# RQLuo/CDLNet-video

Hardware: AMD Instinct MI355X
Metric: Mpix/s denoised (fwd+bwd) at K=30,M=64,P=7 (higher is better)
Workload: dtype f32 (split-bf16 x3 MFMA, fp32 accumulate, fp32 storage)

## Files before the change

cdlnet-video_amd/csrc/cdl_fused2d.hip:

```cpp
#include <atomic>
#include <cstdlib>
#include <type_traits>
#include <mutex>
#include <utility>
#include <vector>

#include "cdl_common.h"
#include "cdl_fused_sweep.h"


namespace {

#include "cdl_wave_dev.h"

typedef __attribute__((ext_vector_type(4))) __bf16 bf16x4;

constexpr int WX = 2;
constexpr int RB = 8;
constexpr int TW = 32 * WX;
constexpr int HALO = 3;
constexpr int RTW = TW + 2 * HALO;
constexpr int RTC = RTW + 2;
constexpr int LDS_W = 32 * 64 * 16;
constexpr int LDS_TAU = 64 * 4;

constexpr int GW_TH = 16;
constexpr int GW_RTH = GW_TH + 2 * HALO;
constexpr int TROWS = GW_RTH + 1;
constexpr int TPITCH = 72;
constexpr int TCOPY = TROWS * TPITCH;
constexpr int WG_THIN_BYTES = 2 * 2 * 4 * TCOPY * 2;
constexpr int IMG_ELEMS = 32 * 32;

template <int WY_>
struct Shape {
    static_assert(WY_ == 2 || WY_ == 4, "64 x 16 or 64 x 32 tiles");
    static constexpr int WY = WY_;
    static constexpr int NW = WX * WY;
    static constexpr int NT = 64 * NW;
    static constexpr int TH = RB * WY;
    static constexpr int RTH = TH + 2 * HALO;
    static constexpr int PITCH = WY == 2 ? 28 : 44;
    static constexpr int COPY = RTC * PITCH;
    static constexpr int LDS_RT = 2 * 4 * COPY * 2;
    static constexpr int SLAB = RTH * RTW;
    static constexpr int LDS_RSUM = 4 * SLAB * 4;
    static constexpr int LDS_TACC = NW * 64 * 4;
    static constexpr int LDS_STAGE = LDS_RT + LDS_RSUM + LDS_W + LDS_TAU + LDS_TACC;
    static constexpr int LDS_DA_THIN = 2 * 4 * TCOPY * 2;
    static constexpr int LDS_DA = LDS_DA_THIN + NW * 2 * 2 * IMG_ELEMS * 2;
    static constexpr int NSTG = (RTH * RTW + NT - 1) / NT;
    static constexpr bool WREG = WY == 2;
};

struct FusedParams {
    const float *r;
    const float *zin;
    unsigned *map;
    float *zout;
    const float *tau;
    float *dtau;
    const uint4 *frags;
    float *patches;
    float sgn;
    int do_synth;
    CDL_DBG_FIELD(int dbg;)
    int N, H, W, tilesX, tilesY;
    int rev;
    const float *r2;
    float *da_partial;
};

__device__ __forceinline__ float embed7(const float *w, int P, int i, int j)
{
    const int off = (7 - P) / 2;
    const int ii = i - off, jj = j - off;
    if (i > 6 || j > 6 || ii < 0 || jj < 0 || ii >= P || jj >= P) return 0.0f;
    return w[ii * P + jj];
}

__device__ __forceinline__ void prep_one(const float *__restrict__ wA, const float *__restrict__ wB,
                                         uint4 *__restrict__ out, int MT, int P, int t)
{
    const int FA = MT * 4, FB = 4 * MT;
    if (t >= (FA + FB) * 64) return;
    const int lane = t & 63, f = t >> 6;
    const int row = lane & 31, h = lane >> 5;
    const int PP = P * P;
    float v[8];
    if (f < FA) {
        const int R = f / 4, ks = f % 4;
        const int ch = 32 * R + row;
#pragma unroll
        for (int jj = 0; jj < 8; ++jj) v[jj] = embed7(wA + (size_t)ch * PP, P, jj, 2 * ks + h);
    } else {
        const int g = f - FA;
        const int Rp = g / (2 * MT), ksB = g % (2 * MT);
        const int R = ksB >> 1, s = ksB & 1;
        const int tap = 32 * Rp + row;
#pragma unroll
        for (int jj = 0; jj < 8; ++jj) {
            const int ch = 32 * R + 16 * s + 8 * (jj >> 2) + 4 * h + (jj & 3);
            v[jj] = embed7(wB + (size_t)ch * PP, P, tap >> 3, tap & 7);
        }
    }
    bf16x8 hi, lo;
#pragma unroll
    for (int jj = 0; jj < 8; ++jj) {
        __bf16 hh = (__bf16)v[jj];
        hi[jj] = hh;
        lo[jj] = (__bf16)(v[jj] - (float)hh);
    }
    uint4 *hi_dst, *lo_dst;
    if (f < FA) { hi_dst = out + (size_t)f * 64; lo_dst = out + (size_t)(FA + f) * 64; }
    else { hi_dst = out + (size_t)(2 * FA + (f - FA)) * 64; lo_dst = out + (size_t)(2 * FA + FB + (f - FA)) * 64; }
    hi_dst[lane] = __builtin_bit_cast(uint4, hi);
    lo_dst[lane] = __builtin_bit_cast(uint4, lo);
}

__global__ void k_prep(const float *__restrict__ wA, const float *__restrict__ wB,
                       uint4 *__restrict__ out, int MT, int P)
{
    prep_one(wA, wB, out, MT, P, blockIdx.x * blockDim.x + threadIdx.x);
}

constexpr int PREP_BATCH = 32;
struct PrepBatch {
    const float *wA[PREP_BATCH];
    const float *wB[PREP_BATCH];
};
__global__ void k_prep_batch(PrepBatch b, uint4 *__restrict__ out, int frag_uint4, int MT, int P)
{
    prep_one(b.wA[blockIdx.y], b.wB[blockIdx.y], out + (size_t)blockIdx.y * frag_uint4, MT, P,
             blockIdx.x * blockDim.x + threadIdx.x);
}

#ifndef CDL_FAT_LD_AUX
#define CDL_FAT_LD_AUX 0
#endif
#ifndef CDL_FAT_ST_AUX
#define CDL_FAT_ST_AUX 0
#endif
__device__ __forceinline__ __amdgpu_buffer_rsrc_t fat_rsrc(const float *base, size_t img_floats)
{
    return __builtin_amdgcn_make_buffer_rsrc(const_cast<float *>(base), 0, (int)(img_floats * 4), 0x00020000);
}
__device__ __forceinline__ float buf_ld(__amdgpu_buffer_rsrc_t r, int voff, int soff)
{
    return __builtin_bit_cast(float, __builtin_amdgcn_raw_buffer_load_b32(r, voff, soff, CDL_FAT_LD_AUX));
}
__device__ __forceinline__ void buf_st(float v, __amdgpu_buffer_rsrc_t r, int voff, int soff)
{
    __builtin_amdgcn_raw_buffer_store_b32(__builtin_bit_cast(unsigned, v), r, voff, soff, CDL_FAT_ST_AUX);
// ... 17 lines not shown
    return __builtin_amdgcn_make_buffer_rsrc(b, 0, __builtin_amdgcn_readfirstlane((int)bytes), 0x00020000);
}

__device__ __forceinline__ float bf16_round(float v) { return (float)(__bf16)v; }

template <int MT>
__device__ __forceinline__ void blk16_load_raw(u32x2 (&z)[MT][4], __amdgpu_buffer_rsrc_t rs, int voff)
{
#pragma unroll
    for (int R = 0; R < MT; ++R)
#pragma unroll
        for (int q = 0; q < 4; ++q)
            z[R][q] = __builtin_bit_cast(u32x2, __builtin_amdgcn_raw_buffer_load_b64(rs, voff, (8 * R + 2 * q) * 32 * 8, CDL_FAT_LD_AUX));
}
__device__ __forceinline__ float blk16_decode(const u32x2 &u, int e)
{
    const unsigned w = (e & 2) ? u.y : u.x;
    return __builtin_bit_cast(float, (e & 1) ? (w & 0xffff0000u) : (w << 16));
}

template <int LAY, int MT>
__device__ __forceinline__ void blk_load(float (&z)[MT][16], __amdgpu_buffer_rsrc_t rs, int voff)
{
    constexpr int EB = LAY == LAY_BLK ? 16 : 8;
#pragma unroll
    for (int R = 0; R < MT; ++R)
#pragma unroll
        for (int q = 0; q < 4; ++q) {
            const int soff = (8 * R + 2 * q) * 32 * EB;
            if constexpr (LAY == LAY_BLK) {
                typedef __attribute__((ext_vector_type(4))) float f32x4;
                const f32x4 f = __builtin_bit_cast(f32x4, __builtin_amdgcn_raw_buffer_load_b128(rs, voff, soff, CDL_FAT_LD_AUX));
                z[R][4 * q + 0] = f.x; z[R][4 * q + 1] = f.y; z[R][4 * q + 2] = f.z; z[R][4 * q + 3] = f.w;
            } else {
                const u32x2 u = __builtin_bit_cast(u32x2, __builtin_amdgcn_raw_buffer_load_b64(rs, voff, soff, CDL_FAT_LD_AUX));
                z[R][4 * q + 0] = __builtin_bit_cast(float, u.x << 16);
                z[R][4 * q + 1] = __builtin_bit_cast(float, u.x & 0xffff0000u);
                z[R][4 * q + 2] = __builtin_bit_cast(float, u.y << 16);
                z[R][4 * q + 3] = __builtin_bit_cast(float, u.y & 0xffff0000u);
            }
        }
}
template <int LAY>
__device__ __forceinline__ void blk_store4(float a0, float a1, float a2, float a3, __amdgpu_buffer_rsrc_t rs, int voff, int quad_pair)
{
    constexpr int EB = LAY == LAY_BLK ? 16 : 8;
    const int soff = quad_pair * 32 * EB;
    if constexpr (LAY == LAY_BLK) {
        typedef __attribute__((ext_vector_type(4))) float f32x4;
        const f32x4 f = {a0, a1, a2, a3};
        __builtin_amdgcn_raw_buffer_store_b128(__builtin_bit_cast(u32x4, f), rs, voff, soff, CDL_FAT_ST_AUX);
    } else {
        u32x2 u;
        u.x = (__builtin_bit_cast(unsigned, a0) >> 16) | (__builtin_bit_cast(unsigned, a1) & 0xffff0000u);
        u.y = (__builtin_bit_cast(unsigned, a2) >> 16) | (__builtin_bit_cast(unsigned, a3) & 0xffff0000u);
        __builtin_amdgcn_raw_buffer_store_b64(u, rs, voff, soff, CDL_FAT_ST_AUX);
    }
}

template <int N>
__device__ __forceinline__ float lane_transpose_sum(const float (&v)[N], int c)
{
    float r = LaneTransposeSum<N>::run(v, c);
    if (N == 16) r += __shfl_xor(r, 16, 64);
    return r;
}

__device__ __forceinline__ float col2im_row(const float (&rv)[4], int h)
{
    const float r4 = upper_half_to_lower(rv[0]);
    const float r5 = upper_half_to_lower(rv[1]);
    const float r6 = upper_half_to_lower(rv[2]);
    const bool lo = h == 0;
    float s = lo ? r6 : 0.0f;
    s = wave_shr1(s) + (lo ? r5 : 0.0f);
    s = wave_shr1(s) + (lo ? r4 : 0.0f);
    s = wave_shr1(s) + (lo ? rv[3] : 0.0f);
    s = wave_shr1(s) + (lo ? rv[2] : 0.0f);
    s = wave_shr1(s) + (lo ? rv[1] : 0.0f);
    s = wave_shr1(s) + (lo ? rv[0] : 0.0f);
    return s;
}

template <int MT, int PREC, int MODE, int LIN, int LOUT, bool DA = false, int WY = 2>
__global__ __launch_bounds__(Shape<WY>::NT) void k_stage(FusedParams p)
{
    using G = Shape<WY>;
    constexpr int NW = G::NW, NT = G::NT, TH = G::TH, RTH = G::RTH, PITCH = G::PITCH, COPY = G::COPY, SLAB = G::SLAB;
    constexpr int LDS_RT = G::LDS_RT, LDS_RSUM = G::LDS_RSUM, LDS_STAGE = G::LDS_STAGE, LDS_DA_THIN = G::LDS_DA_THIN;
    static_assert(!DA || (MODE == MODE_BWD && TH == GW_TH), "dA_k rides in the reverse stage, on k_wgrad2d's 64 x 16 tiles");
    extern __shared__ __attribute__((aligned(16))) unsigned char smem[];
    __bf16 *rt = reinterpret_cast<__bf16 *>(smem);
    float *rsum_all = reinterpret_cast<float *>(smem + LDS_RT);
    const uint4 *wl = reinterpret_cast<const uint4 *>(smem + LDS_RT + LDS_RSUM);
    float *tau_s = reinterpret_cast<float *>(smem + LDS_RT + LDS_RSUM + LDS_W);
    float *tacc_s = tau_s + 64;
    __bf16 *thin2 = reinterpret_cast<__bf16 *>(smem + LDS_STAGE);
    __bf16 *imgs2 = reinterpret_cast<__bf16 *>(smem + LDS_STAGE + LDS_DA_THIN);

    constexpr int M = 32 * MT;
    constexpr int FA = MT * 4, FB = 4 * MT;
    constexpr int NFRAG = (PREC != 1 ? 2 : 1) * (FA + FB);
    constexpr int NSTG = G::NSTG;
    const int tid = threadIdx.x, lane = tid & 63, wid = tid >> 6;
    const int wxi = wid % WX, wyi = wid / WX;
    const int c = lane & 31, h = lane >> 5;
    const size_t HW = (size_t)p.H * p.W;
    const int numTiles = p.N * p.tilesY * p.tilesX;

    {
        uint4 *z4 = reinterpret_cast<uint4 *>(smem);
        for (int i = tid; i < (LDS_RT + LDS_RSUM) / 16; i += NT) z4[i] = make_uint4(0, 0, 0, 0);
        uint4 *wdst = reinterpret_cast<uint4 *>(smem + LDS_RT + LDS_RSUM);
        if (PREC != 1) {
            for (int i = tid; i < NFRAG * 64; i += NT) wdst[i] = p.frags[i];
        } else {
            for (int i = tid; i < FA * 64; i += NT) wdst[i] = p.frags[i];
            for (int i = tid; i < FB * 64; i += NT) wdst[FA * 64 + i] = p.frags[2 * FA * 64 + i];
        }
    }
    float stg[NSTG];
    auto stage_load = [&](int t) {
        int bid = p.rev ? numTiles - 1 - t : t;
        const int txi = bid % p.tilesX; bid /= p.tilesX;
        const int tyi = bid % p.tilesY;
        const int n = bid / p.tilesY;
        const float *rimg = p.r + (size_t)n * HW;
#pragma unroll
        for (int k = 0; k < NSTG; ++k) {
            const int i = tid + k * NT;
            const int yy = i / RTW, xx = i % RTW;
            const int gy = tyi * TH - HALO + yy, gx = txi * TW - HALO + xx;
            float v = 0.0f;
            if (i < RTH * RTW && t < numTiles && !CDL_DBG(p.dbg, 8) && gy >= 0 && gy < p.H && gx >= 0 && gx < p.W)
                v = rimg[(size_t)gy * p.W + gx];
            stg[k] = v;
        }
    };
    auto stage_store = [&]() {
#pragma unroll
        for (int k = 0; k < NSTG; ++k) {
            const int i = tid + k * NT;
            if (i >= RTH * RTW) continue;
            const int yy = i / RTW, xx = i % RTW;
            const __bf16 hh = (__bf16)stg[k];
            const __bf16 ll = (__bf16)(stg[k] - (float)hh);
#pragma unroll
            for (int q = 0; q < 4; ++q)
                if (yy - q >= 0) {
                    rt[(0 * 4 + q) * COPY + xx * PITCH + (yy - q)] = hh;
                    if (PREC != 1) rt[(1 * 4 + q) * COPY + xx * PITCH + (yy - q)] = ll;
                }
        }
    };
    constexpr int NSTG2 = DA ? (GW_RTH * RTW + NT - 1) / NT : 1;
    float stg2[NSTG2];
    auto stage2_load = [&](int t) {
        int bid = p.rev ? numTiles - 1 - t : t;
        const int txi = bid % p.tilesX; bid /= p.tilesX;
        const int tyi = bid % p.tilesY;
        const int n = bid / p.tilesY;
        const float *timg = p.r2 + (t < numTiles ? (size_t)n * HW : 0);
#pragma unroll
        for (int k = 0; k < NSTG2; ++k) {
            const int i = tid + k * NT;
            const int yy = i / RTW, xx = i % RTW;
            const int gy = tyi * TH - HALO + yy, gx = txi * TW - HALO + xx;
            const bool ok = i < GW_RTH * RTW && t < numTiles && gy >= 0 && gy < p.H && gx >= 0 && gx < p.W;
            const float v = timg[ok ? (size_t)gy * p.W + gx : 0];
            stg2[k] = ok ? v : 0.0f;
        }
    };
    auto stage2_store = [&]() {
#pragma unroll
        for (int k = 0; k < NSTG2; ++k) {
            const int i = tid + k * NT;
            if (i >= GW_RTH * RTW) continue;
            const int yy = i / RTW, xx = i % RTW;
            const __bf16 hh = (__bf16)stg2[k];
            const __bf16 ll = (__bf16)(stg2[k] - (float)hh);
#pragma unroll
            for (int sft = 0; sft < 4; ++sft)
                if (xx - sft >= 0) {
                    thin2[(0 * 4 + sft) * TCOPY + yy * TPITCH + xx - sft] = hh;
                    if (PREC != 1) thin2[(1 * 4 + sft) * TCOPY + yy * TPITCH + xx - sft] = ll;
                }
        }
    };
    f32x16 dacc[DA ? MT : 1][2];
    if constexpr (DA) {
#pragma unroll
        for (int R = 0; R < MT; ++R)
#pragma unroll
            for (int tt = 0; tt < 2; ++tt)
#pragma unroll
                for (int v = 0; v < 16; ++v) dacc[R][tt][v] = 0.0f;
        for (int i = tid; i < LDS_DA_THIN / 16; i += NT) reinterpret_cast<uint4 *>(thin2)[i] = make_uint4(0, 0, 0, 0);
        stage2_load(blockIdx.x);
    }
    stage_load(blockIdx.x);
    __syncthreads();
    stage_store();
    if constexpr (DA) stage2_store();

    constexpr int OFF_AH = 0;
    constexpr int OFF_AL = FA;
    constexpr int OFF_BH = (PREC != 1 ? 2 * FA : FA);
    constexpr int OFF_BL = 2 * FA + FB;
    constexpr bool WREG = G::WREG;
    bf16x8 wreg[WREG ? NFRAG : 1];
    if constexpr (WREG) {
#pragma unroll
        for (int f = 0; f < NFRAG; ++f) wreg[f] = __builtin_bit_cast(bf16x8, wl[f * 64 + lane]);
    }
    auto wfrag = [&](int f) __attribute__((always_inline)) {
        if constexpr (WREG) return wreg[f];
        else return __builtin_bit_cast(bf16x8, wl[f * 64 + lane]);
    };

    const int xl = wxi * 32 + c;
    float *rsum = rsum_all + ((wxi & 1) + 2 * (wyi & 1)) * SLAB;
    const bool has_base = (MODE == MODE_FWD) || (MODE == MODE_BWD && p.zin != nullptr);
    const int hw4 = (int)HW * 4;

#pragma unroll 1
    for (int t = blockIdx.x; t < numTiles; t += gridDim.x) {
    const int tile = p.rev ? numTiles - 1 - t : t;
    int bid = tile;
    const int txi = bid % p.tilesX; bid /= p.tilesX;
    const int tyi = bid % p.tilesY;
    const int n = bid / p.tilesY;
    const int tx0 = txi * TW, ty0 = tyi * TH;
    const int x = tx0 + xl;
    if (MODE != MODE_BWD && tid < M) tau_s[tid] = p.tau[(size_t)n * M + tid];
    __syncthreads();
    if (MODE != MODE_BWD) stage_load(t + gridDim.x);

    float ring[7][4];
#pragma unroll
    for (int i = 0; i < 7; ++i)
#pragma unroll
        for (int j = 0; j < 4; ++j) ring[i][j] = 0.0f;
    float tsum[MT * 16];
#pragma unroll
    for (int i = 0; i < MT * 16; ++i) tsum[i] = 0.0f;
    const bool tau_neg = MODE != MODE_BWD && __ballot(lane < M && !(tau_s[lane] >= 0.0f)) != 0ull;
    float taur[MT * 16];
    if (MODE != MODE_BWD) {
#pragma unroll
        for (int R = 0; R < MT; ++R)
#pragma unroll
            for (int qv = 0; qv < 4; ++qv) {
                const float4 t4 = *reinterpret_cast<const float4 *>(&tau_s[32 * R + 8 * qv + 4 * h]);
                taur[16 * R + 4 * qv + 0] = t4.x; taur[16 * R + 4 * qv + 1] = t4.y;
                taur[16 * R + 4 * qv + 2] = t4.z; taur[16 * R + 4 * qv + 3] = t4.w;
            }
    }

    const bool xok = x < p.W;
    const size_t img_in = lay_image_bytes<LIN>(M, p.H, p.W), img_out = lay_image_bytes<LOUT>(M, p.H, p.W);
    const __amdgpu_buffer_rsrc_t rs_in = uniform_rsrc(
        has_base ? (const char *)p.zin + (size_t)n * img_in : (const char *)p.zout, has_base ? img_in : 0);
    unsigned *const map_n = p.map ? p.map + ((size_t)n * 4 + 2 * h) * HW : nullptr;
    const __amdgpu_buffer_rsrc_t rs_out = uniform_rsrc((const char *)p.zout + (size_t)n * img_out, img_out);
    const int lane_off = (int)((4 * h) * HW + x) * 4;
    const int XB = (p.W + 31) / 32, xb = (tx0 >> 5) + wxi;
    constexpr int EB_IN = LIN == LAY_BLK16 ? 8 : 16, EB_OUT = LOUT == LAY_BLK16 ? 8 : 16;
    const int lane_blk_in = (h * 32 + c) * EB_IN, lane_blk_out = (h * 32 + c) * EB_OUT;

#pragma unroll 1
    for (int b = 0; b < RB; ++b) {
        const int yl = wyi * RB + b;
        const int y = ty0 + yl;
        const bool valid = xok && (y < p.H);
        const int voff = valid ? lane_off + y * p.W * 4 : OOB;
        const int blk = (y * XB + xb) * (M / 4) * 32;
        const int voff_in = LIN == LAY_NCHW ? voff : (valid ? blk * EB_IN + lane_blk_in : OOB);
        const int voff_st = CDL_DBG(p.dbg, 1) ? OOB : (LOUT == LAY_NCHW ? voff : (valid ? blk * EB_OUT + lane_blk_out : OOB));

        float zc[MT][16];
        u32x2 zr[MT][4];
        if (MODE != MODE_FIRST && LIN == LAY_BLK16) {
            blk16_load_raw<MT>(zr, rs_in, voff_in);
        } else if (MODE != MODE_FIRST && CDL_DBG(p.dbg, 16)) {
#pragma unroll
            for (int R = 0; R < MT; ++R)
#pragma unroll
                for (int v = 0; v < 16; ++v) zc[R][v] = 0.25f;
        } else if (MODE != MODE_FIRST && LIN != LAY_NCHW) {
            blk_load<LIN, MT>(zc, rs_in, voff_in);
        } else if (MODE != MODE_FIRST) {
#pragma unroll
            for (int R = 0; R < MT; ++R)
#pragma unroll
                for (int v = 0; v < 16; ++v) {
                    const int soff = (32 * R + 8 * (v >> 2) + (v & 3)) * hw4;
                    zc[R][v] = buf_ld(rs_in, voff, soff);
                }
        }
        unsigned sup = 0, sgb = 0;
        if (MODE == MODE_BWD && valid) {
            sup = map_n[(size_t)y * p.W + x];
            sgb = map_n[HW + (size_t)y * p.W + x];
        }

        const int q = b & 3, e = yl - q;
        bf16x8 rh[4], rl[4];
#pragma unroll
        for (int ks = 0; ks < 4; ++ks) {
            const int col = xl + 2 * ks + h;
            const __bf16 *ph = rt + (0 * 4 + q) * COPY + col * PITCH + e;
            const bf16x4 a0 = *reinterpret_cast<const bf16x4 *>(ph);
            const bf16x4 a1 = *reinterpret_cast<const bf16x4 *>(ph + 4);
            rh[ks] = __builtin_shufflevector(a0, a1, 0, 1, 2, 3, 4, 5, 6, 7);
            if (PREC != 1) {
                const __bf16 *pl = rt + (1 * 4 + q) * COPY + col * PITCH + e;
                const bf16x4 b0 = *reinterpret_cast<const bf16x4 *>(pl);
                const bf16x4 b1 = *reinterpret_cast<const bf16x4 *>(pl + 4);
                rl[ks] = __builtin_shufflevector(b0, b1, 0, 1, 2, 3, 4, 5, 6, 7);
            }
        }

        __builtin_amdgcn_sched_barrier(0);
        f32x16 acc[MT];
#pragma unroll
        for (int R = 0; R < MT; ++R)
#pragma unroll
            for (int v = 0; v < 16; ++v) acc[R][v] = 0.0f;
        if CDL_DBG(p.dbg, 4) {
#pragma unroll
            for (int R = 0; R < MT; ++R) acc[R][0] = (float)rh[0][0] + (float)rl[1][1];
        } else {
            bf16x8 wh[2][MT], wlo[2][MT];
#pragma unroll
            for (int R = 0; R < MT; ++R) {
                wh[0][R] = wfrag(OFF_AH + R * 4);
                if (PREC != 1) wlo[0][R] = wfrag(OFF_AL + R * 4);
            }
#pragma unroll
            for (int ks = 0; ks < 4; ++ks) {
                const int cu = ks & 1, nx = cu ^ 1;
                if (ks + 1 < 4) {
#pragma unroll
                    for (int R = 0; R < MT; ++R) {
                        wh[nx][R] = wfrag(OFF_AH + R * 4 + ks + 1);
                        if (PREC != 1) wlo[nx][R] = wfrag(OFF_AL + R * 4 + ks + 1);
                    }
                }
                if (PREC != 1) {
#pragma unroll
                    for (int R = 0; R < MT; ++R) acc[R] = __builtin_amdgcn_mfma_f32_32x32x16_bf16(wlo[cu][R], rh[ks], acc[R], 0, 0, 0);
#pragma unroll
                    for (int R = 0; R < MT; ++R) acc[R] = __builtin_amdgcn_mfma_f32_32x32x16_bf16(wh[cu][R], rl[ks], acc[R], 0, 0, 0);
                    if (PREC == 2) {
#pragma unroll
                        for (int R = 0; R < MT; ++R) acc[R] = __builtin_amdgcn_mfma_f32_32x32x16_bf16(wlo[cu][R], rl[ks], acc[R], 0, 0, 0);
                    }
                }
#pragma unroll
                for (int R = 0; R < MT; ++R) acc[R] = __builtin_amdgcn_mfma_f32_32x32x16_bf16(wh[cu][R], rh[ks], acc[R], 0, 0, 0);
            }
// ... 128 lines not shown
        __builtin_amdgcn_sched_barrier(0);
        f32x16 D[2];
#pragma unroll
        for (int Rp = 0; Rp < 2; ++Rp)
#pragma unroll
            for (int v = 0; v < 16; ++v) D[Rp][v] = 0.0f;
        {
            bf16x8 bwh[2][2], bwl[2][2];
#pragma unroll
            for (int Rp = 0; Rp < 2; ++Rp) {
                bwh[0][Rp] = wfrag(OFF_BH + Rp * 2 * MT);
                if (PREC != 1) bwl[0][Rp] = wfrag(OFF_BL + Rp * 2 * MT);
            }
#pragma unroll
            for (int q = 0; q < 2 * MT; ++q) {
                const int R = q >> 1, s = q & 1, cu = q & 1, nx = cu ^ 1;
                if (q + 1 < 2 * MT) {
#pragma unroll
                    for (int Rp = 0; Rp < 2; ++Rp) {
                        bwh[nx][Rp] = wfrag(OFF_BH + Rp * 2 * MT + q + 1);
                        if (PREC != 1) bwl[nx][Rp] = wfrag(OFF_BL + Rp * 2 * MT + q + 1);
                    }
                }
                bf16x8 zh, zl;
#pragma unroll
                for (int jj = 0; jj < 8; ++jj) {
                    const float val = acc[R][8 * s + jj];
                    const __bf16 hh = (__bf16)val;
                    zh[jj] = hh;
                    if (PREC != 1 && LOUT != LAY_BLK16) zl[jj] = (__bf16)(val - (float)hh);
                }
                if (PREC != 1) {
#pragma unroll
                    for (int Rp = 0; Rp < 2; ++Rp) D[Rp] = __builtin_amdgcn_mfma_f32_32x32x16_bf16(bwl[cu][Rp], zh, D[Rp], 0, 0, 0);
                    if (LOUT != LAY_BLK16) {
#pragma unroll
                        for (int Rp = 0; Rp < 2; ++Rp) D[Rp] = __builtin_amdgcn_mfma_f32_32x32x16_bf16(bwh[cu][Rp], zl, D[Rp], 0, 0, 0);
                        if (PREC == 2) {
#pragma unroll
                            for (int Rp = 0; Rp < 2; ++Rp) D[Rp] = __builtin_amdgcn_mfma_f32_32x32x16_bf16(bwl[cu][Rp], zl, D[Rp], 0, 0, 0);
                        }
                    }
                }
#pragma unroll
                for (int Rp = 0; Rp < 2; ++Rp) D[Rp] = __builtin_amdgcn_mfma_f32_32x32x16_bf16(bwh[cu][Rp], zh, D[Rp], 0, 0, 0);
            }
        }

        __builtin_amdgcn_sched_barrier(0);
#pragma unroll
        for (int Rp = 0; Rp < 2; ++Rp)
#pragma unroll
            for (int v = 0; v < 16; ++v) {
                const int i = 4 * Rp + (v >> 2);
                if (i <= 6) ring[i][v & 3] += D[Rp][v];
            }
        {
            const float cs = col2im_row(ring[0], h);
            if (lane < 38 && !CDL_DBG(p.dbg, 32)) rsum[yl * RTW + 32 * wxi + lane] = cs;
        }
#pragma unroll
        for (int i = 0; i < 6; ++i)
#pragma unroll
            for (int jl = 0; jl < 4; ++jl) ring[i][jl] = ring[i + 1][jl];
#pragma unroll
        for (int jl = 0; jl < 4; ++jl) ring[6][jl] = 0.0f;
    }

    if (MODE != MODE_BWD || p.do_synth) {
#pragma unroll
        for (int i = 0; i < 6; ++i) {
            const float cs = col2im_row(ring[i], h);
            if (lane < 38 && !CDL_DBG(p.dbg, 32)) rsum[(wyi * RB + RB + i) * RTW + 32 * wxi + lane] = cs;
        }
    }
    if (MODE == MODE_BWD) {
        const float tacc = lane_transpose_sum(tsum, c);
        if (c < MT * 16) {
            const int R = c >> 4, v = c & 15;
            tacc_s[wid * 64 + 32 * R + 8 * (v >> 2) + 4 * h + (v & 3)] = tacc;
        }
    }
    __syncthreads();
    if (MODE == MODE_BWD) stage_load(t + gridDim.x);
    if constexpr (DA) stage2_load(t + gridDim.x);
    if (MODE == MODE_BWD && tid < M) {
        float sacc = 0.0f;
#pragma unroll
        for (int w = 0; w < NW; ++w) sacc += tacc_s[w * 64 + tid];
        p.dtau[(size_t)tile * M + tid] = sacc;
    }
    if (MODE != MODE_BWD || p.do_synth) {
        float *patch = p.patches + (size_t)tile * SLAB;
        for (int i = tid; i < SLAB; i += NT) {
            patch[i] = (rsum_all[i] + rsum_all[SLAB + i]) + (rsum_all[2 * SLAB + i] + rsum_all[3 * SLAB + i]);
            rsum_all[i] = 0.0f; rsum_all[SLAB + i] = 0.0f; rsum_all[2 * SLAB + i] = 0.0f; rsum_all[3 * SLAB + i] = 0.0f;
        }
    }
    stage_store();
    if constexpr (DA) stage2_store();
    }
    if constexpr (DA) {
        float *red = reinterpret_cast<float *>(smem);
        for (int w = 0; w < NW; ++w) {
            __syncthreads();
            if (wid == w) {
#pragma unroll
                for (int R = 0; R < MT; ++R)
#pragma unroll
                    for (int tt = 0; tt < 2; ++tt)
#pragma unroll
                        for (int v = 0; v < 16; ++v) {
                            const int ch = 32 * R + (v & 3) + 8 * (v >> 2) + 4 * h;
                            float *dstw = &red[ch * 64 + 32 * tt + c];
                            *dstw = (w == 0 ? 0.0f : *dstw) + dacc[R][tt][v];
                        }
            }
        }
        __syncthreads();
        float *dst = p.da_partial + (size_t)blockIdx.x * 2 * M * 64;
        for (int i = tid; i < M * 64; i += NT) dst[i] = red[i];
    }
}

template <int WY>
__device__ __forceinline__ float patch_sum(const float *__restrict__ patches, int n, int Y, int X,
                                           int tilesX, int tilesY)
{
    constexpr int TH = Shape<WY>::TH, SLAB = Shape<WY>::SLAB;
    const int tyc = Y / TH, txc = X / TW;
    const int ly = Y - tyc * TH, lx = X - txc * TW;
    const int hx = (lx < HALO && txc > 0) ? -1 : ((lx >= TW - HALO && txc + 1 < tilesX) ? 1 : 0);
    const int vy = (ly < HALO && tyc > 0) ? -1 : ((ly >= TH - HALO && tyc + 1 < tilesY) ? 1 : 0);
    const float *own = patches + (((size_t)n * tilesY + tyc) * tilesX + txc) * SLAB + (ly + HALO) * RTW + lx + HALO;
    const ptrdiff_t dx = (ptrdiff_t)hx * (SLAB - TW), dy = (ptrdiff_t)vy * ((ptrdiff_t)tilesX * SLAB - TH * RTW);
    float sum = 0.0f;
    if (vy < 0) {
        if (hx < 0) sum += own[dy + dx];
        sum += own[dy];
        if (hx > 0) sum += own[dy + dx];
    }
    if (hx < 0) sum += own[dx];
    sum += own[0];
    if (hx > 0) sum += own[dx];
    if (vy > 0) {
        if (hx < 0) sum += own[dy + dx];
        sum += own[dy];
        if (hx > 0) sum += own[dy + dx];
    }
    return sum;
}

template <int ASM_ROWS, int WY>
__global__ __launch_bounds__(256) void k_assemble(const float *__restrict__ patches,
                                                  const float *__restrict__ mask,
                                                  const float *__restrict__ sub, float alpha,
                                                  float *__restrict__ out, int N, int H, int W,
                                                  int tilesX, int tilesY, float *__restrict__ acc, int acc_add)
{
    const int X = blockIdx.x * 256 + threadIdx.x, n = blockIdx.z;
    if (X >= W) return;
#pragma unroll
    for (int j = 0; j < ASM_ROWS; ++j) {
        const int Y = blockIdx.y * ASM_ROWS + j;
        if (Y >= H) break;
        const size_t i = ((size_t)n * H + Y) * W + X;
        const float raw = patch_sum<WY>(patches, n, Y, X, tilesX, tilesY);
        if (acc) acc[i] = acc_add ? acc[i] + raw : raw;
        if (!out) continue;
        float sum = alpha * raw;
        if (mask) sum *= mask[i];
        if (sub) sum -= sub[i];
        out[i] = sum;
    }
}

template <int WY>
__global__ __launch_bounds__(256) void k_assemble_v4(const float *__restrict__ patches,
                                                     const float *__restrict__ mask, const float *__restrict__ sub,
// ... 487 lines not shown
}

template <int WY>
int dispatch_stage(const cdl_geom *g, const FusedParams &p, int mode, const Flags &f, hipStream_t st)
{
    dim3 grid((unsigned)stage_grid(g, p));
    if (g->M == 64)
        return f.prec == 0   ? launch_stage<WY, 2, 0>(p, mode, f.lin, f.lout, grid, st)
               : f.prec == 1 ? launch_stage<WY, 2, 1>(p, mode, f.lin, f.lout, grid, st)
                             : launch_stage<WY, 2, 2>(p, mode, f.lin, f.lout, grid, st);
    return f.prec == 0   ? launch_stage<WY, 1, 0>(p, mode, f.lin, f.lout, grid, st)
           : f.prec == 1 ? launch_stage<WY, 1, 1>(p, mode, f.lin, f.lout, grid, st)
                         : launch_stage<WY, 1, 2>(p, mode, f.lin, f.lout, grid, st);
}

int wgrad_grid(const cdl_geom *g)
{
    const size_t tiles = (size_t)g->N * tiles_x(g) * ((g->H + GW_TH - 1) / GW_TH);
    const size_t cus = (size_t)cdl_cu_count();
    return (int)(tiles < cus ? tiles : cus);
}

size_t wgrad_region_floats(const cdl_geom *g) { return (size_t)wgrad_grid(g) * 2 * g->M * 64; }

template <int MT, int PREC, int LAY>
int launch_wgrad_one(const WgradParams &p, int G, hipStream_t st)
{
    const size_t lds = (size_t)WG_THIN_BYTES + (size_t)8 * MT * 2 * IMG_ELEMS * 2;
    if (int rc = cdl_ensure_dynamic_lds((const void *)k_wgrad2d<MT, PREC, LAY>, (int)lds)) return rc;
    k_wgrad2d<MT, PREC, LAY><<<G, 512, lds, st>>>(p);
    CDL_LAUNCH_CHECK();
    return 0;
}

template <int MT, int PREC>
int launch_wgrad(const WgradParams &p, int lay, int G, hipStream_t st)
{
    if (lay == LAY_BLK) return launch_wgrad_one<MT, PREC, LAY_BLK>(p, G, st);
    if (lay == LAY_BLK16) return launch_wgrad_one<MT, PREC, LAY_BLK16>(p, G, st);
    return launch_wgrad_one<MT, PREC, LAY_NCHW>(p, G, st);
}

inline size_t larger(size_t a, size_t b) { return a > b ? a : b; }
template <int WY> inline size_t shape_tiles(const cdl_geom *g) { return (size_t)g->N * tiles_x(g) * tiles_y<WY>(g); }

template <int WY>
FusedParams stage_params(const cdl_geom *g, const Flags &f, const void *frags, float *patches)
{
    FusedParams p = {};
    p.rev = f.rev;
    p.frags = reinterpret_cast<const uint4 *>(frags);
    p.patches = patches; CDL_DBG_FIELD(p.dbg = debug_flags();)
    p.N = g->N; p.H = g->H; p.W = g->W;
    p.tilesX = tiles_x(g); p.tilesY = tiles_y<WY>(g);
    return p;
}

template <int WY>
int iter_fwd(const cdl_geom *g, const float *r, const float *zin, const float *tau, const void *frags, float sgn,
             float *zout, float *patches, unsigned *map_out, int precision, void *stream)
{
    if (!fused_shape_ok(g)) return CDL_EUNSUPPORTED;
    if (!r || !tau || !frags || !zout || !patches || zout == zin) return CDL_EINVAL;
    if (!cdl_aligned16(frags, patches)) return CDL_EUNSUPPORTED;
    const Flags f = parse_flags(precision);
    if (!f.ok) return CDL_EINVAL;
    if ((f.lin && !cdl_aligned16(zin)) || (f.lout && !cdl_aligned16(zout))) return CDL_EUNSUPPORTED;
    FusedParams p = stage_params<WY>(g, f, frags, patches);
    p.r = r; p.zin = zin; p.zout = zout; p.tau = tau; p.map = map_out;
    p.sgn = sgn; p.do_synth = 1;
    return dispatch_stage<WY>(g, p, zin ? MODE_FWD : MODE_FIRST, f, S(stream));
}

int launch_wgrad_reduce(const cdl_geom *g, const WgradReduce &job, hipStream_t st)
{
    k_wgrad_reduce<<<wgrad_reduce_blocks(job, g->M, g->Ph), 1024, 0, st>>>(job, g->M, g->Ph);
    CDL_LAUNCH_CHECK();
    return 0;
}

template <int WY>
int stage_bwd(const cdl_geom *g, const float *thin, const float *base, const unsigned *map, const void *frags,
              float *du_out, float *patches, float *dtau_partial, int do_synth, int precision, const float *r2,
              float alpha, float *dA, float *workspace, void *stream, WgradReduce *defer = nullptr)
{
    if (!fused_shape_ok(g)) return CDL_EUNSUPPORTED;
    if (!thin || !map || !frags || !du_out || !dtau_partial || du_out == base) return CDL_EINVAL;
    if (!cdl_aligned16(frags, patches)) return CDL_EUNSUPPORTED;
    if (do_synth && !patches) return CDL_EINVAL;
    if (r2 && (!dA || !workspace)) return CDL_EINVAL;
    const Flags f = parse_flags(precision);
    if (!f.ok) return CDL_EINVAL;
    if ((f.lin && !cdl_aligned16(base)) || (f.lout && !cdl_aligned16(du_out))) return CDL_EUNSUPPORTED;
    FusedParams p = stage_params<WY>(g, f, frags, patches);
    p.r = thin; p.zin = base; p.map = const_cast<unsigned *>(map); p.zout = du_out; p.dtau = dtau_partial;
    p.sgn = 1.0f; p.do_synth = do_synth ? 1 : 0;
    p.r2 = r2; p.da_partial = workspace;
    int rc = dispatch_stage<WY>(g, p, MODE_BWD, f, S(stream));
    if (rc || !r2) return rc;
    const WgradReduce job = {workspace, stage_grid(g, p), dA, nullptr, alpha, 0.0f, 0};
    if (defer) { *defer = job; return 0; }
    return launch_wgrad_reduce(g, job, S(stream));
}

int wgrad_partials(const cdl_geom *g, const float *X0, const float *T0, float alpha0, float *dw0,
                   const float *X1, const float *T1, float alpha1, float *dw1, float *workspace,
                   int precision, void *stream, WgradReduce *job)
{
    if (!fused_shape_ok(g)) return CDL_EUNSUPPORTED;
    if (!workspace || (!X0 && !X1)) return CDL_EINVAL;
    if ((X0 && (!T0 || !dw0)) || (X1 && (!T1 || !dw1))) return CDL_EINVAL;
    const Flags f = parse_flags(precision);
    if (!f.ok) return CDL_EINVAL;
    if (f.lin && !cdl_aligned16(X0, X1)) return CDL_EUNSUPPORTED;
    WgradParams p = {};
    p.rev = f.rev;
    p.X[0] = X0; p.T[0] = T0; p.X[1] = X1; p.T[1] = T1;
    p.single = (X0 != nullptr) != (X1 != nullptr);
    if (p.single) {
        if (!X0) { X0 = X1; T0 = T1; alpha0 = alpha1; dw0 = dw1; X1 = nullptr; }
        p.X[0] = p.X[1] = X0; p.T[0] = p.T[1] = T0;
    }
    p.partial = workspace;
    p.N = g->N; p.H = g->H; p.W = g->W;
    p.tilesX = tiles_x(g); p.tilesY = (g->H + GW_TH - 1) / GW_TH;
    p.numTiles = p.N * p.tilesX * p.tilesY;
    int G = wgrad_grid(g);
    if (p.single && G > (p.numTiles + 1) / 2) G = (p.numTiles + 1) / 2;
    int rc;
    if (g->M == 64)
        rc = f.prec == 0 ? launch_wgrad<2, 0>(p, f.lin, G, S(stream))
             : f.prec == 1 ? launch_wgrad<2, 1>(p, f.lin, G, S(stream)) : launch_wgrad<2, 2>(p, f.lin, G, S(stream));
    else
        rc = f.prec == 0 ? launch_wgrad<1, 0>(p, f.lin, G, S(stream))
             : f.prec == 1 ? launch_wgrad<1, 1>(p, f.lin, G, S(stream)) : launch_wgrad<1, 2>(p, f.lin, G, S(stream));
    if (rc) return rc;
    *job = WgradReduce{workspace, G, X0 ? dw0 : nullptr, X1 ? dw1 : nullptr, alpha0, alpha1, p.single};
    return 0;
}

template <int WY>
int assemble(const cdl_geom *g, const float *patches, const float *mask, const float *sub, float alpha, float *out,
             float *acc, int acc_add, void *stream)
{
    if (!fused_shape_ok(g)) return CDL_EUNSUPPORTED;
    if (!patches || (!out && !acc)) return CDL_EINVAL;
    const int tx = tiles_x(g), ty = tiles_y<WY>(g);
    if ((size_t)g->N * g->H * g->W >= ((size_t)1 << 20) && cdl_assemble16(g->W, out, mask, sub, acc)) {
        dim3 grid((unsigned)((g->W + 255) / 256), (unsigned)((g->H + 7) / 8), (unsigned)g->N);
        k_assemble_v4<WY><<<grid, 256, 0, S(stream)>>>(patches, mask, sub, alpha, out, g->N, g->H, g->W, tx, ty, acc, acc_add);
        CDL_LAUNCH_CHECK();
    } else if ((size_t)g->N * g->H * g->W >= ((size_t)1 << 20)) {
        dim3 grid((unsigned)((g->W + 255) / 256), (unsigned)((g->H + 3) / 4), (unsigned)g->N);
        k_assemble<4, WY><<<grid, 256, 0, S(stream)>>>(patches, mask, sub, alpha, out, g->N, g->H, g->W, tx, ty, acc, acc_add);
        CDL_LAUNCH_CHECK();
    } else {
        dim3 grid((unsigned)((g->W + 255) / 256), (unsigned)g->H, (unsigned)g->N);
        k_assemble<1, WY><<<grid, 256, 0, S(stream)>>>(patches, mask, sub, alpha, out, g->N, g->H, g->W, tx, ty, acc, acc_add);
        CDL_LAUNCH_CHECK();
    }
    return 0;
}

struct TimingState {
    std::mutex mu;
    std::atomic<bool> on{false};
    struct Pair { hipEvent_t start, stop; int cls, dev; };
    std::vector<Pair> pairs;
    std::vector<std::pair<hipEvent_t, int>> spare;
};
TimingState g_timing;

struct TimingScope {
    hipStream_t st;
    hipEvent_t stop = nullptr;
    TimingScope(int c, hipStream_t s) : st(s)
    {
        if (!g_timing.on.load(std::memory_order_relaxed)) return;
        std::lock_guard<std::mutex> lk(g_timing.mu);
        const int dev = cdl_current_device();
// ... 8 lines not shown
        }
        (void)hipEventRecord(ev[0], st);
        stop = ev[1];
        g_timing.pairs.push_back({ev[0], ev[1], c, dev});
    }
    ~TimingScope()
    {
        if (stop) (void)hipEventRecord(stop, st);
    }
};

int prep_pairs(const float *const *w1, const float *const *w2, int K, int shift2, void *frags, int M, int P,
               hipStream_t st)
{
    if (!cdl_aligned16(frags)) return CDL_EUNSUPPORTED;
    const int MT = M / 32, threads = 8 * MT * 64;
    const int frag_uint4 = (int)(cdl_fused2d_frag_bytes(M) / 16);
    for (int k0 = 0; k0 < K; k0 += PREP_BATCH) {
        PrepBatch b;
        const int nb = cdl_pair_batch(&b, w1, w2, K, shift2, k0);
        dim3 grid((unsigned)((threads + 255) / 256), (unsigned)nb);
        k_prep_batch<<<grid, 256, 0, st>>>(b, reinterpret_cast<uint4 *>(frags) + (size_t)k0 * frag_uint4, frag_uint4, MT, P);
        CDL_LAUNCH_CHECK();
    }
    return 0;
}

int snake_enabled() { return cdl_opts().fused_snake; }

template <int WY>
int forward_sweep(const cdl_geom *g, int K, const float *yp, const float *mask, const float *tau,
                  const float *const *wA, const float *const *wB, float *const *z, float *const *r,
                  unsigned *const *maps, float *xp, void *frags, float *patches, const Flags &f, void *stream)
{
    const size_t nm = (size_t)g->N * g->M;
    const int L = f.lin;
    int rc = prep_pairs(wA, wB, K, 1, frags, g->M, g->Ph, S(stream));
    if (rc) return rc;
    return cdl_forward_order_sweep(
        K, frags, cdl_fused2d_frag_bytes(g->M), yp, mask, yp, 1.0f, r, xp, snake_enabled(), L, LAY_NCHW,
        [&](int k, const void *fk, const float *thin, bool reversed, int, int lay_out) {
            TimingScope ts(k ? 0 : 3, S(stream));
            return iter_fwd<WY>(g, thin, k ? z[k - 1] : nullptr, tau + k * nm, fk, k ? -1.0f : 1.0f, z[k], patches, maps ? maps[k] : nullptr,
                                f.prec | CDL_LAYOUT_IN(L) | CDL_LAYOUT_OUT(lay_out) | (reversed ? CDL_TILES_REVERSED : 0), stream);
        },
        [&](const float *m, const float *sub, float alpha, float *out) {
            return assemble<WY>(g, patches, m, sub, alpha, out, nullptr, 0, stream);
        });
}

template <int WY>
int backward_sweep(const cdl_geom *g, int K, const float *yp, const float *mask, const float *c,
                   const float *const *wA, const float *const *wB, const float *const *z,
                   const float *const *r, const unsigned *const *maps, const float *g_xp,
                   const float *g_z, float *const *dA,
                   float *const *dB, float *dt, float *du0, float *du1, float *q, void *frags,
                   float *patches, float *dtau_partial, float *wgrad_ws, const Flags &f, float *dyp,
                   float *dtau, void *stream)
{
    const int M = g->M;
    float *du[2] = {du0, du1};
    const int L = f.lin;
    const int sdir = snake_enabled() ? (((K - 1) & 1) ? CDL_TILES_REVERSED : 0) : 0;
    const int wdir = snake_enabled() ? (sdir ^ CDL_TILES_REVERSED) : 0;
    const int sprec = f.prec | sdir, wprec = f.prec | wdir;
    int rc = cdl_fused2d_wgrad(g, z[K - 1], g_xp, 1.0f, dB[0], nullptr, nullptr, 0.0f, nullptr, wgrad_ws,
                               wprec, stream);
    if (rc) return rc;
    const float *thin = g_xp, *base = g_z;
    const size_t fb = cdl_fused2d_frag_bytes(M);
    rc = prep_pairs(wB, wA, K, 0, frags, M, g->Ph, S(stream));
    if (rc) return rc;
    float *ws_a = wgrad_ws, *ws_b = wgrad_ws + wgrad_region_floats(g);
    const int per_img = tiles_x(g) * tiles_y<WY>(g);
    for (int k = K - 1, flip = 0; k >= 0; --k, flip ^= 1) {
        const void *fk = static_cast<const char *>(frags) + (size_t)k * fb;
        float *duk = du[flip];
        const bool ride = Shape<WY>::TH == GW_TH && cdl_opts().fused_da;
        SweepReduce red = {};
        {
            TimingScope ts(1, S(stream));
            rc = stage_bwd<WY>(g, thin, base, maps[k], fk, duk, patches, dtau_partial, k >= 1 || dyp,
                               sprec | CDL_LAYOUT_IN(k == K - 1 ? LAY_NCHW : L) | CDL_LAYOUT_OUT(L),
                               ride ? (k >= 1 ? r[k - 1] : yp) : nullptr, k >= 1 ? -1.0f : 1.0f, dA[k], ws_a, stream, &red.w[0]);
        }
        if (rc) return rc;
        if (ride) red.wblocks[0] = wgrad_reduce_blocks(red.w[0], M, g->Ph);
        red.t = DtauReduce{dtau_partial, c, dt + (size_t)k * 2 * M, dt + (size_t)k * 2 * M + M, g->N, per_img};
        if (dtau) {
            rc = cdl_dtau_per_sample(dtau_partial, g->N, M, per_img, (size_t)per_img * M, 1, M, dtau + (size_t)k * g->N * M, stream);
            if (rc) return rc;
        }
        if (k == 0 && dyp) {
            rc = assemble<WY>(g, patches, nullptr, nullptr, 1.0f, nullptr, dyp, K > 1, stream);
            if (rc) return rc;
        }
        if (k >= 1) {
            rc = assemble<WY>(g, patches, mask, nullptr, -1.0f, q, dyp, k < K - 1, stream);
            if (rc) return rc;
            {
                TimingScope ts(2, S(stream));
                rc = ride ? wgrad_partials(g, z[k - 1], q, 1.0f, dB[k], nullptr, nullptr, 0.0f, nullptr, ws_b,
                                           wprec | CDL_LAYOUT_IN(L), stream, &red.w[1])
                          : wgrad_partials(g, duk, r[k - 1], -1.0f, dA[k], z[k - 1], q, 1.0f, dB[k], ws_b,
                                           wprec | CDL_LAYOUT_IN(L), stream, &red.w[1]);
            }
            thin = q;
        } else if (!ride) {
            rc = wgrad_partials(g, duk, yp, 1.0f, dA[0], nullptr, nullptr, 0.0f, nullptr, ws_b, wprec | CDL_LAYOUT_IN(L), stream,
                                &red.w[1]);
        }
        if (rc) return rc;
        if (k >= 1 || !ride) red.wblocks[1] = wgrad_reduce_blocks(red.w[1], M, g->Ph);
        k_sweep_reduce<<<red.wblocks[0] + red.wblocks[1] + (M + 3) / 4, 1024, 0, S(stream)>>>(red, M, g->Ph);
        CDL_LAUNCH_CHECK();
        base = duk;
    }
    return 0;
}

template <int WY>
int tangent_sweep(const cdl_geom *g, int K, const float *vp, const float *nvp, const float *mask,
                  const float *const *wA, const float *const *wB, const unsigned *const *maps, float *const *zd,
                  float *const *nrd, float *xdp, void *frags, float *patches, float *dtau_partial, const Flags &f,
                  void *stream)
{
    int rc = prep_pairs(wA, wB, K, 1, frags, g->M, g->Ph, S(stream));
    if (rc) return rc;
    return cdl_forward_order_sweep(
        K, frags, cdl_fused2d_frag_bytes(g->M), vp, mask, nvp, -1.0f, nrd, xdp, snake_enabled(), f.lin, LAY_NCHW,
        [&](int k, const void *fk, const float *thin, bool reversed, int lay_in, int lay_out) {
            return stage_bwd<WY>(g, thin, k ? zd[k - 1] : nullptr, maps[k], fk, zd[k], patches, dtau_partial, 1,
                                 f.prec | CDL_LAYOUT_IN(lay_in) | CDL_LAYOUT_OUT(lay_out) | (reversed ? CDL_TILES_REVERSED : 0),
                                 nullptr, 0.0f, nullptr, nullptr, stream);
        },
        [&](const float *m, const float *sub, float alpha, float *out) {
            return assemble<WY>(g, patches, m, sub, alpha, out, nullptr, 0, stream);
        });
}

}

extern "C" {

int cdl_fused2d_supported(const cdl_geom *g) { return fused_shape_ok(g) ? 1 : 0; }

size_t cdl_fused2d_frag_bytes(int M) { return (size_t)2 * (M / 32) * 8 * 64 * 16; }

size_t cdl_fused2d_patch_floats(const cdl_geom *g)
{
    if (!fused_shape_ok(g)) return 0;
    return larger(shape_tiles<2>(g) * Shape<2>::SLAB, shape_tiles<4>(g) * Shape<4>::SLAB);
}

size_t cdl_fused2d_tiles(const cdl_geom *g)
{
    if (!fused_shape_ok(g)) return 0;
    return larger(shape_tiles<2>(g), shape_tiles<4>(g));
}

int cdl_fused2d_prep(const float *wA, const float *wB, void *frags, int M, int P, void *stream)
{
    if (!wA || !wB || !frags || (M != 32 && M != 64) || P < 1 || P > 7 || !(P & 1)) return CDL_EINVAL;
    if (!cdl_aligned16(frags)) return CDL_EUNSUPPORTED;
    const int MT = M / 32, threads = 8 * MT * 64;
    k_prep<<<(threads + 255) / 256, 256, 0, S(stream)>>>(wA, wB, reinterpret_cast<uint4 *>(frags), MT, P);
    CDL_LAUNCH_CHECK();
// ... 159 lines not shown
```

Before: 120.6.

## Stage halo tiles as per-thread runs, vectorize patch writes, skip dead du output

Tile staging now gives each thread a contiguous run of 8 pixels along one column (or row, for the dA thin tile). The four shifted bf16 copies are then written with packed 2- and 4-element LDS stores instead of scattered scalar stores. In backward with WY==2 the next tile's loads, including the dA stage2 loads, are now issued ahead of the main compute loop rather than after it. Patch reduction and zeroing now use float4 vectors for WY==2, and a drop_zout flag skips writing du at k==0 when dA rides in the reverse stage, since that output is unused. Loading ahead holds more values in registers across the loop, which risks higher register pressure and lower occupancy.

```diff
diff --git a/cdlnet-video_amd/csrc/cdl_fused2d.hip b/cdlnet-video_amd/csrc/cdl_fused2d.hip
--- a/cdlnet-video_amd/csrc/cdl_fused2d.hip
+++ b/cdlnet-video_amd/csrc/cdl_fused2d.hip
@@ -49,7 +49,6 @@
     static constexpr int LDS_STAGE = LDS_RT + LDS_RSUM + LDS_W + LDS_TAU + LDS_TACC;
     static constexpr int LDS_DA_THIN = 2 * 4 * TCOPY * 2;
     static constexpr int LDS_DA = LDS_DA_THIN + NW * 2 * 2 * IMG_ELEMS * 2;
-    static constexpr int NSTG = (RTH * RTW + NT - 1) / NT;
     static constexpr bool WREG = WY == 2;
 };
 
@@ -69,6 +68,7 @@
     int rev;
     const float *r2;
     float *da_partial;
+    int drop_zout;
 };
 
 __device__ __forceinline__ float embed7(const float *w, int P, int i, int j)
@@ -252,6 +252,41 @@
     return s;
 }
 
+constexpr int RUN = 8;
+typedef __attribute__((ext_vector_type(2))) __bf16 bf16x2;
+template <int S>
+__device__ __forceinline__ void store_run(__bf16 *dst, const __bf16 (&v)[RUN], bool low)
+{
+    static_assert(S >= 0 && S <= 3, "four shifted copies");
+    if (!low) {
+        if constexpr (S == 1) dst[-1] = v[0];
+        if constexpr (S == 2) *reinterpret_cast<bf16x2 *>(dst - 2) = bf16x2{v[0], v[1]};
+        if constexpr (S == 3) { dst[-3] = v[0]; *reinterpret_cast<bf16x2 *>(dst - 2) = bf16x2{v[1], v[2]}; }
+    }
+    *reinterpret_cast<bf16x4 *>(dst) = bf16x4{v[S], v[S + 1], v[S + 2], v[S + 3]};
+    if constexpr (S == 0) *reinterpret_cast<bf16x4 *>(dst + 4) = bf16x4{v[4], v[5], v[6], v[7]};
+    if constexpr (S == 1) { *reinterpret_cast<bf16x2 *>(dst + 4) = bf16x2{v[5], v[6]}; dst[6] = v[7]; }
+    if constexpr (S == 2) *reinterpret_cast<bf16x2 *>(dst + 4) = bf16x2{v[6], v[7]};
+    if constexpr (S == 3) dst[4] = v[7];
+}
+template <int PREC>
+__device__ __forceinline__ void store_run_copies(__bf16 *dst, int copy_elems, const float (&f)[RUN], bool low)
+{
+    __bf16 hh[RUN], ll[RUN];
+#pragma unroll
+    for (int j = 0; j < RUN; ++j) {
+        hh[j] = (__bf16)f[j];
+        ll[j] = (__bf16)(f[j] - (float)hh[j]);
+    }
+    store_run<0>(dst, hh, low); store_run<1>(dst + copy_elems, hh, low);
+    store_run<2>(dst + 2 * copy_elems, hh, low); store_run<3>(dst + 3 * copy_elems, hh, low);
+    if (PREC != 1) {
+        dst += 4 * copy_elems;
+        store_run<0>(dst, ll, low); store_run<1>(dst + copy_elems, ll, low);
+        store_run<2>(dst + 2 * copy_elems, ll, low); store_run<3>(dst + 3 * copy_elems, ll, low);
+    }
+}
+
 template <int MT, int PREC, int MODE, int LIN, int LOUT, bool DA = false, int WY = 2>
 __global__ __launch_bounds__(Shape<WY>::NT) void k_stage(FusedParams p)
 {
@@ -271,7 +306,6 @@
     constexpr int M = 32 * MT;
     constexpr int FA = MT * 4, FB = 4 * MT;
     constexpr int NFRAG = (PREC != 1 ? 2 : 1) * (FA + FB);
-    constexpr int NSTG = G::NSTG;
     const int tid = threadIdx.x, lane = tid & 63, wid = tid >> 6;
     const int wxi = wid % WX, wyi = wid / WX;
     const int c = lane & 31, h = lane >> 5;
@@ -289,72 +323,56 @@
             for (int i = tid; i < FB * 64; i += NT) wdst[FA * 64 + i] = p.frags[2 * FA * 64 + i];
         }
     }
-    float stg[NSTG];
+    constexpr int RT_RUNS = (RTH + RUN - 1) / RUN;
+    static_assert(RTW * RT_RUNS <= NT && RT_RUNS * RUN <= PITCH, "one run per thread; a column's runs stay inside its pitch");
+    const int rt_xx = tid % RTW, rt_y0 = (tid / RTW) * RUN;
+    const bool rt_on = tid < RTW * RT_RUNS;
+    __bf16 *const rt_dst = rt + rt_xx * PITCH + rt_y0;
+    float stg[RUN];
     auto stage_load = [&](int t) {
         int bid = p.rev ? numTiles - 1 - t : t;
         const int txi = bid % p.tilesX; bid /= p.tilesX;
         const int tyi = bid % p.tilesY;
         const int n = bid / p.tilesY;
         const float *rimg = p.r + (size_t)n * HW;
-#pragma unroll
-        for (int k = 0; k < NSTG; ++k) {
-            const int i = tid + k * NT;
-            const int yy = i / RTW, xx = i % RTW;
-            const int gy = tyi * TH - HALO + yy, gx = txi * TW - HALO + xx;
+        const int gy0 = tyi * TH - HALO + rt_y0, gx = txi * TW - HALO + rt_xx;
+        const bool colok = rt_on && t < numTiles && !CDL_DBG(p.dbg, 8) && gx >= 0 && gx < p.W;
+#pragma unroll
+        for (int j = 0; j < RUN; ++j) {
+            const int gy = gy0 + j;
             float v = 0.0f;
-            if (i < RTH * RTW && t < numTiles && !CDL_DBG(p.dbg, 8) && gy >= 0 && gy < p.H && gx >= 0 && gx < p.W)
-                v = rimg[(size_t)gy * p.W + gx];
-            stg[k] = v;
+            if (colok && rt_y0 + j < RTH && gy >= 0 && gy < p.H) v = rimg[(size_t)gy * p.W + gx];
+            stg[j] = v;
         }
     };
     auto stage_store = [&]() {
-#pragma unroll
-        for (int k = 0; k < NSTG; ++k) {
-            const int i = tid + k * NT;
-            if (i >= RTH * RTW) continue;
-            const int yy = i / RTW, xx = i % RTW;
-            const __bf16 hh = (__bf16)stg[k];
-            const __bf16 ll = (__bf16)(stg[k] - (float)hh);
-#pragma unroll
-            for (int q = 0; q < 4; ++q)
-                if (yy - q >= 0) {
-                    rt[(0 * 4 + q) * COPY + xx * PITCH + (yy - q)] = hh;
-                    if (PREC != 1) rt[(1 * 4 + q) * COPY + xx * PITCH + (yy - q)] = ll;
-                }
-        }
+        if (rt_on) store_run_copies<PREC>(rt_dst, COPY, stg, rt_y0 == 0);
     };
-    constexpr int NSTG2 = DA ? (GW_RTH * RTW + NT - 1) / NT : 1;
-    float stg2[NSTG2];
+    constexpr int T2_RUNS = (RTW + RUN - 1) / RUN;
+    static_assert(!DA || (GW_RTH * T2_RUNS <= NT && T2_RUNS * RUN <= TPITCH), "one run per thread; a row's runs stay inside its pitch");
+    const int t2_x0 = (tid % T2_RUNS) * RUN, t2_yy = tid / T2_RUNS;
+    const bool t2_on = tid < GW_RTH * T2_RUNS;
+    __bf16 *const t2_dst = thin2 + t2_yy * TPITCH + t2_x0;
+    float stg2[DA ? RUN : 1];
     auto stage2_load = [&](int t) {
         int bid = p.rev ? numTiles - 1 - t : t;
         const int txi = bid % p.tilesX; bid /= p.tilesX;
         const int tyi = bid % p.tilesY;
         const int n = bid / p.tilesY;
         const float *timg = p.r2 + (t < numTiles ? (size_t)n * HW : 0);
-#pragma unroll
-        for (int k = 0; k < NSTG2; ++k) {
-            const int i = tid + k * NT;
-            const int yy = i / RTW, xx = i % RTW;
-            const int gy = tyi * TH - HALO + yy, gx = txi * TW - HALO + xx;
-            const bool ok = i < GW_RTH * RTW && t < numTiles && gy >= 0 && gy < p.H && gx >= 0 && gx < p.W;
+        const int gy = tyi * TH - HALO + t2_yy, gx0 = txi * TW - HALO + t2_x0;
+        const bool rowok = t2_on && t < numTiles && !CDL_DBG(p.dbg, 8) && gy >= 0 && gy < p.H;
+#pragma unroll
+        for (int j = 0; j < (DA ? RUN : 1); ++j) {
+            const int gx = gx0 + j;
+            const bool ok = rowok && t2_x0 + j < RTW && gx >= 0 && gx < p.W;
             const float v = timg[ok ? (size_t)gy * p.W + gx : 0];
-            stg2[k] = ok ? v : 0.0f;
+            stg2[j] = ok ? v : 0.0f;
         }
     };
     auto stage2_store = [&]() {
-#pragma unroll
-        for (int k = 0; k < NSTG2; ++k) {
-            const int i = tid + k * NT;
-            if (i >= GW_RTH * RTW) continue;
-            const int yy = i / RTW, xx = i % RTW;
-            const __bf16 hh = (__bf16)stg2[k];
-            const __bf16 ll = (__bf16)(stg2[k] - (float)hh);
-#pragma unroll
-            for (int sft = 0; sft < 4; ++sft)
-                if (xx - sft >= 0) {
-                    thin2[(0 * 4 + sft) * TCOPY + yy * TPITCH + xx - sft] = hh;
-                    if (PREC != 1) thin2[(1 * 4 + sft) * TCOPY + yy * TPITCH + xx - sft] = ll;
-                }
+        if constexpr (DA) {
+            if (t2_on) store_run_copies<PREC>(t2_dst, TCOPY, stg2, t2_x0 == 0);
         }
     };
     f32x16 dacc[DA ? MT : 1][2];
@@ -404,7 +422,11 @@
     const int x = tx0 + xl;
     if (MODE != MODE_BWD && tid < M) tau_s[tid] = p.tau[(size_t)n * M + tid];
     __syncthreads();
-    if (MODE != MODE_BWD) stage_load(t + gridDim.x);
+    constexpr bool LOAD_AHEAD = MODE != MODE_BWD || WY == 2;
+    if (LOAD_AHEAD) {
+        stage_load(t + gridDim.x);
+        if constexpr (DA) stage2_load(t + gridDim.x);
+    }
 
     float ring[7][4];
 #pragma unroll
@@ -446,7 +468,7 @@
         const int voff = valid ? lane_off + y * p.W * 4 : OOB;
         const int blk = (y * XB + xb) * (M / 4) * 32;
         const int voff_in = LIN == LAY_NCHW ? voff : (valid ? blk * EB_IN + lane_blk_in : OOB);
-        const int voff_st = CDL_DBG(p.dbg, 1) ? OOB : (LOUT == LAY_NCHW ? voff : (valid ? blk * EB_OUT + lane_blk_out : OOB));
+        const int voff_st = (CDL_DBG(p.dbg, 1) || (MODE == MODE_BWD && p.drop_zout)) ? OOB : (LOUT == LAY_NCHW ? voff : (valid ? blk * EB_OUT + lane_blk_out : OOB));
 
         float zc[MT][16];
         u32x2 zr[MT][4];
@@ -741,19 +763,24 @@
         }
     }
     __syncthreads();
-    if (MODE == MODE_BWD) stage_load(t + gridDim.x);
-    if constexpr (DA) stage2_load(t + gridDim.x);
+    if (!LOAD_AHEAD) stage_load(t + gridDim.x);
     if (MODE == MODE_BWD && tid < M) {
         float sacc = 0.0f;
 #pragma unroll
         for (int w = 0; w < NW; ++w) sacc += tacc_s[w * 64 + tid];
         p.dtau[(size_t)tile * M + tid] = sacc;
     }
+    if CDL_DBG(p.dbg, 128) continue;
     if (MODE != MODE_BWD || p.do_synth) {
-        float *patch = p.patches + (size_t)tile * SLAB;
-        for (int i = tid; i < SLAB; i += NT) {
-            patch[i] = (rsum_all[i] + rsum_all[SLAB + i]) + (rsum_all[2 * SLAB + i] + rsum_all[3 * SLAB + i]);
-            rsum_all[i] = 0.0f; rsum_all[SLAB + i] = 0.0f; rsum_all[2 * SLAB + i] = 0.0f; rsum_all[3 * SLAB + i] = 0.0f;
+        typedef __attribute__((ext_vector_type(4))) float f32x4;
+        using PV = std::conditional_t<WY == 2, f32x4, float>;
+        constexpr int NV = SLAB * 4 / (int)sizeof(PV);
+        static_assert(SLAB * 4 % sizeof(PV) == 0 && LDS_RT % sizeof(PV) == 0, "slabs and patches are whole vectors");
+        PV *patch = reinterpret_cast<PV *>(p.patches + (size_t)tile * SLAB);
+        PV *rs = reinterpret_cast<PV *>(rsum_all);
+        for (int i = tid; i < NV; i += NT) {
+            patch[i] = (rs[i] + rs[NV + i]) + (rs[2 * NV + i] + rs[3 * NV + i]);
+            rs[i] = (PV)(0.0f); rs[NV + i] = (PV)(0.0f); rs[2 * NV + i] = (PV)(0.0f); rs[3 * NV + i] = (PV)(0.0f);
         }
     }
     stage_store();
@@ -1407,7 +1434,7 @@
 template <int WY>
 int stage_bwd(const cdl_geom *g, const float *thin, const float *base, const unsigned *map, const void *frags,
               float *du_out, float *patches, float *dtau_partial, int do_synth, int precision, const float *r2,
-              float alpha, float *dA, float *workspace, void *stream, WgradReduce *defer = nullptr)
+              float alpha, float *dA, float *workspace, void *stream, WgradReduce *defer = nullptr, bool drop_out = false)
 {
     if (!fused_shape_ok(g)) return CDL_EUNSUPPORTED;
     if (!thin || !map || !frags || !du_out || !dtau_partial || du_out == base) return CDL_EINVAL;
@@ -1421,6 +1448,7 @@
     p.r = thin; p.zin = base; p.map = const_cast<unsigned *>(map); p.zout = du_out; p.dtau = dtau_partial;
     p.sgn = 1.0f; p.do_synth = do_synth ? 1 : 0;
     p.r2 = r2; p.da_partial = workspace;
+    p.drop_zout = drop_out ? 1 : 0;
     int rc = dispatch_stage<WY>(g, p, MODE_BWD, f, S(stream));
     if (rc || !r2) return rc;
     const WgradReduce job = {workspace, stage_grid(g, p), dA, nullptr, alpha, 0.0f, 0};
@@ -1595,7 +1623,8 @@
             TimingScope ts(1, S(stream));
             rc = stage_bwd<WY>(g, thin, base, maps[k], fk, duk, patches, dtau_partial, k >= 1 || dyp,
                                sprec | CDL_LAYOUT_IN(k == K - 1 ? LAY_NCHW : L) | CDL_LAYOUT_OUT(L),
-                               ride ? (k >= 1 ? r[k - 1] : yp) : nullptr, k >= 1 ? -1.0f : 1.0f, dA[k], ws_a, stream, &red.w[0]);
+                               ride ? (k >= 1 ? r[k - 1] : yp) : nullptr, k >= 1 ? -1.0f : 1.0f, dA[k], ws_a, stream, &red.w[0],
+                               ride && k == 0);
         }
         if (rc) return rc;
         if (ride) red.wblocks[0] = wgrad_reduce_blocks(red.w[0], M, g->Ph);
```

Measured after the change: 123.4 (median of 6 runs). +2.3%, better.
